# ProjectZKM/Ziren

Measured on AMD Instinct MI355X. Metric: shard-proofs/sec, higher is better.
Workload: dtype u32

## Files before the change

ziren_amd/csrc/host_ctx.hpp:

```cpp
#pragma once
static thread_local std::string g_err;

#define HIP_CHECK(expr)                                                                          \
  do {                                                                                           \
    hipError_t _e = (expr);                                                                      \
    if (_e != hipSuccess)                                                                        \
      throw std::runtime_error(std::string(#expr) + ": " + hipGetErrorString(_e) + " (" + __FILE__ + ":" + \
                               std::to_string(__LINE__) + ")");                                  \
  } while (0)
#define LAUNCH_CHECK() HIP_CHECK(hipGetLastError())
#define KLAUNCH(ctx, name, bytes, kernel, grid, block, lds, ...)                                        \
  do {                                                                                                   \
    (ctx)->flush_staged();                                                                               \
    if ((ctx)->kbegin(name, (double)(bytes))) {                                                          \
       \
      hipExtLaunchKernelGGL(kernel, grid, block, lds, (ctx)->cur, (ctx)->krecs.back().start,             \
                            (ctx)->krecs.back().stop, 0, __VA_ARGS__);                                   \
    } else {                                                                                             \
      hipLaunchKernelGGL(kernel, grid, block, lds, (ctx)->cur, __VA_ARGS__);                             \
    }                                                                                                    \
    LAUNCH_CHECK();                                                                                      \
  } while (0)

static inline int log2_strict(size_t n) {
// ... 78 lines not shown
  static constexpr size_t UP_SLAB_BYTES = (size_t)32 << 20;
  hipStream_t cur = nullptr;
  hipStream_t ev_dma = nullptr;
  struct Prefetched { size_t bytes; hipEvent_t landed; };
  std::map<const void*, Prefetched> prefetched;
  const uint32_t* events_on_device(const void* events, size_t bytes, uint32_t** owned) {
    *owned = nullptr;
    auto it = prefetched.find(events);
    if (it != prefetched.end()) {
      if (bytes > it->second.bytes) throw std::runtime_error("zkm_tracegen: more events asked for than zkm_events_upload_async copied");
      HIP_CHECK(hipStreamWaitEvent(stream, it->second.landed, 0));
      return (const uint32_t*)events;
    }
    uint32_t* d = (uint32_t*)alloc(std::max<size_t>(bytes, 4));
    *owned = d;
    if (bytes) HIP_CHECK(hipMemcpyAsync(d, events, bytes, hipMemcpyHostToDevice, stream));
    return d;
  }
  std::mutex mu;
  std::multimap<size_t, void*> free_list;
  std::map<void*, size_t> live;
  std::map<int, uint32_t*> tw_fwd, tw_inv;
  std::vector<std::pair<std::string, hipEvent_t>> marks;
  std::vector<hipEvent_t> event_pool;
  std::vector<std::string> timing_names;
  std::vector<float> timing_ms;
  struct KRec { const char* name; double bytes; hipEvent_t start, stop; };
  struct KStat { double ms = 0, bytes = 0; uint32_t calls = 0; };
  std::vector<KRec> krecs;
  std::map<std::string, KStat> kstats;
  int kernel_timing = 2;
  bool lde_overlap = !(getenv("ZKM_LDE_OVERLAP") && atoi(getenv("ZKM_LDE_OVERLAP")) == 0);
  bool rows_up_front = !(getenv("ZKM_ROWS_UP_FRONT") && atoi(getenv("ZKM_ROWS_UP_FRONT")) == 0);
  bool root_poll = !(getenv("ZKM_ROOT_POLL") && atoi(getenv("ZKM_ROOT_POLL")) == 0);
  int root_spin_before_yield = getenv("ZKM_ROOT_SPIN") ? atoi(getenv("ZKM_ROOT_SPIN")) : 4096;
  int root_sleep_ns = getenv("ZKM_ROOT_SLEEP_NS") ? atoi(getenv("ZKM_ROOT_SLEEP_NS")) : 0;
  bool host_wait_blocking = getenv("ZKM_HOST_WAIT") && !strcmp(getenv("ZKM_HOST_WAIT"), "blocking");
  int wait_sleep_ns = getenv("ZKM_WAIT_SLEEP_NS") ? atoi(getenv("ZKM_WAIT_SLEEP_NS")) : 20000;
  struct TimerSlack {
    long saved = -1;
    void tighten() {
      if (saved >= 0) return;
      saved = prctl(PR_GET_TIMERSLACK, 0, 0, 0, 0);
      if (saved >= 0) prctl(PR_SET_TIMERSLACK, 1000UL, 0, 0, 0);
    }
    ~TimerSlack() { if (saved >= 0) prctl(PR_SET_TIMERSLACK, (unsigned long)saved, 0, 0, 0); }
  };
  static void sleep_ns(long ns, TimerSlack& slack) {
    slack.tighten();
    timespec ts{0, ns};
    nanosleep(&ts, nullptr);
  }
  void sync(hipStream_t s) {
    if (!host_wait_blocking) { HIP_CHECK(hipStreamSynchronize(s)); return; }
    TimerSlack slack;
    for (int i = 0;; i++) {
      const hipError_t e = hipStreamQuery(s);
      if (e == hipSuccess) return;
      if (e != hipErrorNotReady) HIP_CHECK(e);
      if (i >= 4) sleep_ns(wait_sleep_ns, slack);
    }
  }
  std::map<uint64_t, std::vector<hipFunction_t>> quotient_fns;
  std::map<uint64_t, hipFunction_t> quotient_uniform_fns;
  std::map<uint64_t, hipFunction_t> perm_fns;
  std::vector<hipModule_t> modules;
// ... 345 lines not shown
```

ziren_amd/csrc/host_open.hpp:

```cpp
#pragma once
static E4 host_pow2k(E4 a, int k) { return kb::epow2k(a, k); }

struct Writer {
  uint32_t* dst;
  size_t cap, n = 0;
  Writer(uint32_t* d, size_t c) : dst(d), cap(d ? c : 0) {}
  void u(uint32_t v) { if (n < cap) dst[n] = v; n++; }
  void words(const uint32_t* p, size_t cnt) {
    if (n < cap) memcpy(dst + n, p, std::min(cnt, cap - n) * 4);
    n += cnt;
  }
  void ext(const E4& e) { words(e.c, 4); }
  size_t size() const { return n; }
};

struct RoundMat {
  const uint32_t* evals; size_t n; size_t width; uint32_t shift;
  const zkm_matrix* lde;
  int n_points;
  std::vector<E4> y[2];
  size_t col0 = 0;
};
struct Round { const zkm_pcs_data* data; std::vector<RoundMat> mats; };

// ... 121 lines not shown
    KLAUNCH(ctx, "scan", 0.0, stark::scan_totals, dim3((unsigned)(4 * scans.size())), dim3(stark::THREADS), 0, d);
    KLAUNCH(ctx, "scan", bytes, stark::scan_add_offsets, dim3(scans.back().blk_end), dim3(stark::THREADS), 0, d);
  }
}

struct ShardOpening {
  struct Loose {
    zkm_ctx* ctx;
    std::vector<void*> v;
    void disown(void* p) { v.erase(std::remove(v.begin(), v.end(), p), v.end()); }
    ~Loose() { for (void* p : v) ctx->release(p); }
  };
  struct Guard { zkm_ctx* c; std::vector<zkm_pcs_data*> d; ~Guard() { for (auto p : d) free_pcs_data(c, p); } };

  zkm_ctx* ctx;
  const zkm_pk* pk;
  zkm_main_data* md;
  const zkm_fri_config* fri;
  uint32_t num_pv_elts;
  zkm_challenger* ch;
  hipStream_t st;
  const int bl;
  const size_t nc;
  std::vector<ChipMeta> chips;
  Loose loose;
  std::vector<void*>& scratch;
  Guard guard;
  E4 perm_ch[2];
  uint32_t* d_pv = nullptr;
  std::vector<zkm_matrix> perm_traces;
  std::vector<E4> local_sums;
  std::vector<std::array<uint32_t, 14>> global_sums;
  zkm_pcs_data* perm_data = nullptr;
  std::vector<zkm_matrix> qchunks;
  std::vector<uint32_t> qshifts;
  zkm_pcs_data* quot_data = nullptr;
  E4 zeta;
  std::vector<Round> rounds;
  int log_max = 0;
  std::vector<E4*> ro = std::vector<E4*>(32, nullptr);
  const uint32_t** col_ptr_lde = nullptr;
  const uint32_t** col_ptr_eval = nullptr;
  uint32_t* col_mask = nullptr;
  std::vector<E4*> layers;
  std::vector<Tree> ftrees;
  std::vector<std::array<uint32_t, 8>> commits;
  E4 final_poly;
  uint32_t pow_witness = 0;
  std::vector<size_t> indices;
  const uint32_t* gathered = nullptr;
  std::vector<uint32_t> gathered_big;

  void* salloc(size_t bytes) { void* p = ctx->alloc(bytes); scratch.push_back(p); return p; }

  ShardOpening(zkm_ctx* ctx_, const zkm_pk* pk_, zkm_main_data* md_, const zkm_chip_desc* chips_in, const zkm_fri_config* fri_, uint32_t num_pv_elts_,
               zkm_challenger* ch_)
      : ctx(ctx_), pk(pk_), md(md_), fri(fri_), num_pv_elts(num_pv_elts_), ch(ch_), st(ctx_->stream), bl((int)fri_->log_blowup), nc(md_->order.size()),
        loose{ctx_, {}}, scratch(loose.v), guard{ctx_, {}} {
  for (size_t i = 0; i < nc; i++) chips.push_back(chip_meta(&chips_in[md->order[i]], md->traces[i].h, md->public_values.size()));
  for (size_t i = 0; i < nc; i++) {
    if (chips[i].desc->main_width != md->traces[i].w) throw std::runtime_error("chip main_width does not match its trace");
    if ((int)chips[i].desc->log_quotient_degree > bl) throw std::runtime_error("log_quotient_degree > log_blowup unsupported");
    if (chips[i].desc->prep_index >= 0 && (!pk->data || (size_t)chips[i].desc->prep_index >= pk->prep.size()))
      throw std::runtime_error("chip references a preprocessed trace the proving key does not hold");
  }
  if (bl < 1 || bl > 4) throw std::runtime_error("fri.log_blowup out of range (1..4)");
// ... 26 lines not shown
      if (chips[i].perm_ext_w > 0) d_blobs[i] = (uint32_t*)ctx->upload_staged(chips[i].desc->lookups, chips[i].desc->lookups_len * 4, &scratch);
    for (size_t i = 0; i < nc; i++) {
      const ChipMeta& c = chips[i];
      zkm_matrix& pt = perm_traces[i];
      pt.h = c.n; pt.w = (size_t)c.perm_ext_w * 4;
      pt.d = ctx->alloc_n<uint32_t>(std::max<size_t>(pt.h * pt.w, 1));
      scratch.push_back(pt.d);
      if (c.perm_ext_w > 0) {
        const uint32_t* prep = c.desc->prep_index >= 0 ? pk->prep[c.desc->prep_index].d : nullptr;
        launch_permutation_trace(ctx, c, (const uint32_t*)d_blobs[i], (const uint32_t*)md->traces[i].d, prep, perm_ch[0], (const E4*)d_bp, pt,
                                 [&](size_t bytes) { return salloc(bytes); }, scans);
        uint32_t* last = pt.d + (size_t)(c.perm_ext_w - 1) * 4 * c.n;
        for (int e = 0; e < 4; e++) sum_src.push_back(last + (size_t)e * c.n + (c.n - 1));
      } else {
        for (int e = 0; e < 4; e++) sum_src.push_back(nullptr);
      }
      if (c.desc->commit_scope_global) {
        const zkm_matrix& m = md->traces[i];
        for (int k = 0; k < 14; k++) sum_src.push_back(m.d + (m.w - 14 + k) * m.h + (m.h - 1));
      } else {
        for (int k = 0; k < 14; k++) sum_src.push_back(nullptr);
      }
    }
    launch_scans(ctx, scans, &scratch);
    const uint32_t* d_zero = (const uint32_t*)ctx->upload_staged("\0\0\0\0", 4, &scratch);
    for (auto& p : sum_src) if (!p) p = d_zero;
    const uint32_t** d_sum_src = (const uint32_t**)ctx->upload_staged(sum_src.data(), sum_src.size() * sizeof(void*), &scratch);
    uint32_t* d_sums = (uint32_t*)salloc(sum_src.size() * 4);
    KLAUNCH(ctx, "gather_words", 0.0, open::gather_words, dim3(div_up(sum_src.size(), open::THREADS)), dim3(open::THREADS), 0,
            (const uint32_t* const*)d_sum_src, sum_src.size(), d_sums);
    h_sums = ctx->download_async(d_sums, sum_src.size());
  }
  ctx->mark("permutation traces");
  perm_data = pcs_commit(ctx, perm_traces, {}, bl);
  guard.d.push_back(perm_data);
  perm_data->owned_evals = perm_traces;
  for (auto& m : perm_traces) loose.disown(m.d);
  ctx->mark("commit permutation");
  for (size_t i = 0; i < nc; i++) {
    for (int e = 0; e < 4; e++) local_sums[i].c[e] = h_sums[18 * i + e];
    if (chips[i].desc->commit_scope_global) {
      for (int k = 0; k < 14; k++) global_sums[i][k] = h_sums[18 * i + 4 + k];
    } else {
      for (int k = 0; k < 7; k++) { global_sums[i][k] = kb::to_monty(SEPTIC_X[k]); global_sums[i][7 + k] = kb::to_monty(SEPTIC_Y[k]); }
    }
  }
  chal::observe_slice(ch, perm_data->root, 8);
  for (size_t i = 0; i < nc; i++) {
    chal::observe_ext(ch, local_sums[i]);
    chal::observe_slice(ch, global_sums[i].data(), 14);
  }
  }

  void quotient_phase() {
  E4 alpha = chal::sample_ext(ch);
  std::vector<std::function<void()>> launches;
  for (size_t i = 0; i < nc; i++) {
    const ChipMeta& c = chips[i];
    const zkm_chip_desc* d = c.desc;
    int lqd = d->log_quotient_degree;
    int lq = c.log_n + lqd;
    size_t Q = (size_t)1 << lq;
    size_t nchunks = (size_t)1 << lqd;
    uint32_t* qbuf = ctx->alloc_n<uint32_t>(Q * 4);
    scratch.push_back(qbuf);
    size_t C = d->num_constraints;
    std::vector<E4> ap(std::max<size_t>(C, 1));
    E4 p = kb::eone();
    for (size_t k = 0; k < C; k++) { ap[C - 1 - k] = p; p = kb::emul(p, alpha); }
    E4* d_ap = (E4*)ctx->upload_staged(ap.data(), ap.size() * sizeof(E4), &scratch);
    uint32_t consts[32] = {0};
    for (int k = 0; k < 14; k++) consts[k] = global_sums[i][k];
    uint32_t w_q = kb::two_adic_generator(lq);
    uint32_t s_pow_n = kb::pow(kb::GEN, (uint64_t)c.n);
    uint32_t wr = kb::two_adic_generator(lqd), wp = kb::ONE;
    for (size_t k = 0; k < nchunks; k++) {
      consts[16 + k] = kb::sub(kb::mul(s_pow_n, wp), kb::ONE);
      consts[24 + k] = kb::inv(consts[16 + k]);
      wp = kb::mul(wp, wr);
    }
    uint32_t* d_consts = (uint32_t*)ctx->upload_staged(consts, sizeof consts, &scratch);
    static const uint32_t empty_prog[4] = {0, 1, 0, 1};
    uint32_t* d_prog = (uint32_t*)ctx->upload_staged(d->program_len ? d->program : empty_prog, std::max<size_t>(d->program_len, 4) * 4, &scratch);
    stark::QuotientArgs a;
    a.program = d_prog + 4;
    a.n_instr = d->program_len ? d->program[0] : 0;
    a.n_regs = d->program_len ? d->program[1] : 1;
    a.main_lde = md->data->ldes[i].d; a.main_stride = md->data->ldes[i].h;
    a.prep_lde = d->prep_index >= 0 ? pk->data->ldes[d->prep_index].d : nullptr;
    a.prep_stride = d->prep_index >= 0 ? pk->data->ldes[d->prep_index].h : 0;
    a.perm_lde = perm_data->ldes[i].d; a.perm_stride = perm_data->ldes[i].h;
    a.log_n = c.log_n; a.lqd = lqd;
    a.alpha_pows = d_ap; a.public_values = d_pv;
    a.perm_alpha = perm_ch[0]; a.perm_beta = perm_ch[1];
    a.local_sum = local_sums[i];
    a.consts = d_consts;
    a.w_q = w_q; a.g_inv = kb::inv(kb::two_adic_generator(c.log_n));
    a.out = qbuf;
// ... 4 lines not shown
    while (per_thread * bd > 64 * 1024 && bd > 64) bd >>= 1;
    size_t lds = per_thread * bd;
    if (lds > 152 * 1024) throw std::runtime_error(std::string("constraint program of chip ") + d->name + " needs too many registers");
    double qbytes = 4.0 * Q * (d->main_width + d->prep_width + 4.0 * c.perm_ext_w) + 16.0 * Q;
    auto fit = d->program_len ? ctx->quotient_fns.find(fnv1a(d->program, d->program_len)) : ctx->quotient_fns.end();
    const bool special = fit != ctx->quotient_fns.end();
    const std::vector<hipFunction_t>* fns = special ? &fit->second : nullptr;
    hipFunction_t uni_fn = nullptr;
    a.uniforms = nullptr;
    if (special) {
      auto uit = ctx->quotient_uniform_fns.find(fit->first);
      if (uit != ctx->quotient_uniform_fns.end()) {
        uni_fn = uit->second;
        a.uniforms = ctx->alloc_n<uint32_t>(stark::QUOTIENT_UNIFORM_WORDS);
        scratch.push_back(a.uniforms);
      }
    }
    launches.push_back([this, a, fns, uni_fn, Q, bd, lds, qbytes]() mutable {
      if (fns) {
        size_t arg_size = sizeof(a);
        void* config[] = {HIP_LAUNCH_PARAM_BUFFER_POINTER, &a, HIP_LAUNCH_PARAM_BUFFER_SIZE, &arg_size, HIP_LAUNCH_PARAM_END};
        ctx->flush_staged();
        if (uni_fn)
          HIP_CHECK(hipExtModuleLaunchKernel(uni_fn, 64, 1, 1, 64, 1, 1, 0, st, nullptr, config, nullptr, nullptr, 0));
        for (hipFunction_t fn : *fns) {
          const bool timed = ctx->kbegin("quotient", qbytes);
          HIP_CHECK(hipExtModuleLaunchKernel(fn, div_up(Q, 256) * 256, 1, 1, 256, 1, 1, 0, st, nullptr, config,
                                             timed ? ctx->krecs.back().start : nullptr, timed ? ctx->krecs.back().stop : nullptr, 0));
        }
      } else {
        KLAUNCH(ctx, "quotient", qbytes, stark::quotient_kernel, dim3(div_up(Q, bd)), dim3(bd), lds, a);
      }
    });
    uint32_t wqp = kb::ONE;
    for (size_t k = 0; k < nchunks; k++) {
      zkm_matrix m; m.h = c.n; m.w = 4; m.d = qbuf + k * 4 * c.n; m.owned = (k == 0);
      qchunks.push_back(m);
      qshifts.push_back(kb::mul(kb::GEN, wqp));
      wqp = kb::mul(wqp, w_q);
    }
    if (i == 0) { launches[0](); launches[0] = [] {}; }
  }
  for (auto& l : launches) l();
  ctx->mark("quotient values");
  quot_data = pcs_commit(ctx, qchunks, qshifts, bl);
  for (auto& m : qchunks) if (m.owned) { quot_data->owned_evals.push_back(m); loose.disown(m.d); }
  guard.d.push_back(quot_data);
  ctx->mark("commit quotient");
  chal::observe_slice(ch, quot_data->root, 8);
  zeta = chal::sample_ext(ch);
  }

  void opened_values() {
  if (pk->data) {
    Round r; r.data = pk->data;
    for (size_t j = 0; j < pk->prep.size(); j++)
      r.mats.push_back(RoundMat{pk->prep[j].d, pk->prep[j].h, pk->prep[j].w, kb::ONE, &pk->data->ldes[j], pk->local_only[j] ? 1 : 2, {}});
    rounds.push_back(r);
  }
  {
    Round r; r.data = md->data;
    for (size_t i = 0; i < nc; i++)
      r.mats.push_back(RoundMat{md->traces[i].d, md->traces[i].h, md->traces[i].w, kb::ONE, &md->data->ldes[i], chips[i].desc->local_only ? 1 : 2, {}});
    rounds.push_back(r);
    Round rp; rp.data = perm_data;
    for (size_t i = 0; i < nc; i++)
      rp.mats.push_back(RoundMat{perm_traces[i].d, perm_traces[i].h, perm_traces[i].w, kb::ONE, &perm_data->ldes[i], 2, {}});
    rounds.push_back(rp);
    Round rq; rq.data = quot_data;
    for (size_t i = 0; i < qchunks.size(); i++)
      rq.mats.push_back(RoundMat{qchunks[i].d, qchunks[i].h, 4, qshifts[i], &quot_data->ldes[i], 1, {}});
    rounds.push_back(rq);
  }
// ... 373 lines not shown
```

ziren_amd/csrc/host_pcs.hpp:

```cpp
#pragma once
struct LdeJob {
  const uint32_t* in; size_t n, w; uint32_t lde_shift; uint32_t* out;
  uint32_t* cflag = nullptr;
  bool uniform = false;
};

static void lde_batch_chunk(zkm_ctx* ctx, const std::vector<LdeJob>& jobs, int bl) {
  std::vector<size_t> order(jobs.size());
  std::iota(order.begin(), order.end(), 0);
  std::stable_sort(order.begin(), order.end(), [&](size_t a, size_t b) { return jobs[a].n > jobs[b].n; });
  std::vector<lde::Batch> hb(1);
  lde::Batch& b = hb[0];
  memset(&b, 0, sizeof b);
  b.log_blowup = bl;
  const size_t cosets = (size_t)1 << bl;
  size_t tmp1_words = 0, tmp2_words = 0;
  for (size_t oi : order) if (jobs[oi].n > ((size_t)1 << lde::LOG_ROW_MAX)) { tmp1_words += jobs[oi].n * jobs[oi].w; tmp2_words += (jobs[oi].n * jobs[oi].w) << bl; }
  uint32_t* tmp1 = tmp1_words ? ctx->alloc_n<uint32_t>(tmp1_words) : nullptr;
  uint32_t* tmp2 = tmp2_words ? ctx->alloc_n<uint32_t>(tmp2_words) : nullptr;
  size_t t1 = 0, t2 = 0;
  size_t big_cols = 0, fc = 0;
  for (size_t oi : order) if (jobs[oi].n > ((size_t)1 << lde::LOG_ROW_MAX) && !jobs[oi].cflag) big_cols += jobs[oi].w;
  uint32_t* cflags = big_cols ? ctx->alloc_n<uint32_t>(2 * big_cols) : nullptr;
  if (cflags) HIP_CHECK(hipMemsetAsync(cflags, 0, 2 * big_cols * sizeof(uint32_t), ctx->cur));
  uint32_t blk[4] = {0, 0, 0, 0};
  size_t lds_cols = 0, lds_small = 0;
  double bytes_inv = 0, bytes_rows = 0, bytes_fwd = 0, bytes_small = 0;
  int nm = 0;
  for (size_t p = 0; p < order.size();) {
    const size_t n = jobs[order[p]].n;
    const int k = log2_strict(n);
    const int lb = std::min(k, lde::LOG_ROW_MAX), la = k - lb;
    lde::Group& g = b.g[b.n_groups];
    g.la = la; g.lb = lb;
    g.logT = la ? std::min(14 - la, lb) : 0;
    g.first_mat = nm;
    g.w_N = kb::two_adic_generator(k + bl);
    g.n_inv = kb::inv(kb::to_monty((uint32_t)(n % kb::P)));
    g.twb_inv = lb > 0 ? ctx->twiddles(lb, true) : nullptr;
    g.twb_fwd = lb > 0 ? ctx->twiddles(lb, false) : nullptr;
    if (la) {
      g.twa_inv = ctx->twiddles_ct(la, true);
      g.twa_fwd = ctx->twiddles_ct(la, false);
      auto pw = ctx->pow_tables(k);
      g.pw_lo = pw.first; g.pw_hi = pw.second;
      g.tw_rows = ctx->row_twiddles(k);
    }
    uint32_t cols = 0;
    for (; p < order.size() && jobs[order[p]].n == n; p++) {
      const LdeJob& j = jobs[order[p]];
      lde::Mat& m = b.m[nm++];
      m.in = j.in; m.out = j.out; m.col0 = cols; m.w = (uint32_t)j.w; m.shift = j.lde_shift; m.uniform = j.uniform ? 1u : 0u;
      if (la) {
        m.tmp1 = tmp1 + t1; t1 += n * j.w;
        m.tmp2 = tmp2 + t2; t2 += (n * j.w) << bl;
        if (j.cflag) m.cflag = j.cflag;
        else { m.cflag = cflags + fc; fc += 2 * j.w; }
        auto ct = ctx->coset_tables(k, bl, j.lde_shift);
        m.twf = ct.twf; m.cs = ct.cs;
      }
      cols += (uint32_t)j.w;
    }
    g.n_cols = cols;
    g.n_mats = nm - g.first_mat;
    const double cells = (double)n * cols;
    if (la) {
      const size_t per_col = ((size_t)1 << lb) >> g.logT;
      blk[lde::K_COLS_INV] += (uint32_t)(per_col * cols);
      blk[lde::K_ROWS_BIG] += (uint32_t)(((size_t)1 << la) * cols);
      blk[lde::K_COLS_FWD] += (uint32_t)(per_col * cols * cosets);
      lds_cols = std::max(lds_cols, ((size_t)1 << la) * (((size_t)1 << g.logT) + 1) * 4);
      bytes_inv += 8.0 * cells; bytes_rows += 4.0 * cells * (1 + cosets); bytes_fwd += 8.0 * cells * cosets;
      for (int mi = (int)g.first_mat; mi < nm; mi++) if (b.m[mi].uniform) bytes_inv -= 8.0 * (double)n * b.m[mi].w;
    } else {
      blk[lde::K_ROWS_SMALL] += cols;
      const size_t B = (size_t)1 << lb;
      lds_small = std::max(lds_small, (2 * (B + (B >> 5)) + 64 + (B > 64 ? (B >> 6) : 1)) * 4);
      bytes_small += 4.0 * cells * (1 + cosets);
    }
    for (int q = 0; q < 4; q++) g.blk_end[q] = blk[q];
    b.n_groups++;
  }
  const lde::Batch* d = (const lde::Batch*)ctx->upload_staged(&b, sizeof b);
  if (blk[lde::K_COLS_INV]) {
    constexpr size_t B = (size_t)1 << lde::LOG_ROW_MAX;
    const size_t big_lds = (B + (B >> 5)) * 4;
    KLAUNCH(ctx, "lde_cols_inverse", bytes_inv, lde::lde_cols<false>, dim3(blk[lde::K_COLS_INV]), dim3(lde::THREADS), lds_cols, d);
    KLAUNCH(ctx, "lde_rows", bytes_rows, lde::lde_rows_big, dim3(blk[lde::K_ROWS_BIG]), dim3(lde::THREADS), big_lds, d);
    KLAUNCH(ctx, "lde_cols_forward", bytes_fwd, lde::lde_cols<true>, dim3(blk[lde::K_COLS_FWD]), dim3(lde::THREADS), lds_cols, d);
  }
  if (blk[lde::K_ROWS_SMALL])
    KLAUNCH(ctx, "lde_rows", bytes_small, lde::lde_rows, dim3(blk[lde::K_ROWS_SMALL]), dim3(lde::THREADS), lds_small, d);
  ctx->release_here(tmp1);
  ctx->release_here(tmp2);
  ctx->release_here(cflags);
  ctx->release_here((void*)d);
}

static void lde_batch(zkm_ctx* ctx, const std::vector<LdeJob>& all, int bl) {
  constexpr size_t SCRATCH_BUDGET_WORDS = ((size_t)12 << 30) / 4;
  std::vector<LdeJob> jobs;
  size_t scratch = 0;
  for (auto& j : all) {
    if (j.w == 0) continue;
    const size_t need = j.n > ((size_t)1 << lde::LOG_ROW_MAX) ? j.n * j.w + ((j.n * j.w) << bl) : 0;
    if (!jobs.empty() && ((int)jobs.size() == lde::MAX_MATS || scratch + need > SCRATCH_BUDGET_WORDS)) { lde_batch_chunk(ctx, jobs, bl); jobs.clear(); scratch = 0; }
    jobs.push_back(j);
    scratch += need;
  }
  if (!jobs.empty()) lde_batch_chunk(ctx, jobs, bl);
}

static void lde_columns(zkm_ctx* ctx, const uint32_t* in, size_t n, size_t w, int bl, uint32_t lde_shift, uint32_t* out) {
  lde_batch(ctx, {LdeJob{in, n, w, lde_shift, out}}, bl);
}

static const uint32_t** upload_ptrs(zkm_ctx* ctx, const std::vector<const uint32_t*>& ptrs) {
  return (const uint32_t**)ctx->upload_staged(ptrs.data(), ptrs.size() * sizeof(void*));
}

static bool compress_small_layer(zkm_ctx* ctx, Tree& t, int layer, size_t len, merkle::DevChallenger* d_ch = nullptr, kb::E4* d_beta = nullptr,
                                 uint32_t* h_root_slot = nullptr) {
  static const size_t LANES_MAX = getenv("ZKM_LANES_MAX") ? (size_t)atol(getenv("ZKM_LANES_MAX")) : 4096;
  const size_t TAIL = 64;
  if (len > LANES_MAX) {
    KLAUNCH(ctx, "compress_layer", 96.0 * len, merkle::compress_layer, dim3(div_up(len, merkle::THREADS)), dim3(merkle::THREADS), 0,
            (const uint32_t*)(t.digests + t.layer_off[layer] * 8), t.digests + t.layer_off[layer + 1] * 8, len,
            (const uint32_t* const*)nullptr, 0, (const uint32_t*)nullptr);
    return false;
  }
  if (len <= TAIL) {
    uint32_t* h_root = h_root_slot ? h_root_slot : (uint32_t*)ctx->pin_alloc(32);
    if (h_root) for (int k = 0; k < 8; k++) ((volatile uint32_t*)h_root)[k] = 0xffffffffu;
    KLAUNCH(ctx, "compress_tail", 96.0 * len, merkle::compress_tail_lanes, dim3(1), dim3(1024), 0, t.digests + t.layer_off[layer] * 8, len, h_root, d_ch, d_beta);
    t.h_root = h_root;
    return true;
  }
  KLAUNCH(ctx, "compress_small", 96.0 * len, merkle::compress_layer_lanes, dim3(div_up(len * 16, merkle::THREADS)), dim3(merkle::THREADS),
          0, (const uint32_t*)(t.digests + t.layer_off[layer] * 8), t.digests + t.layer_off[layer + 1] * 8, len);
  return false;
}

static inline void cpu_relax() {
#if defined(__x86_64__) || defined(__i386__)
  __builtin_ia32_pause();
#elif defined(__aarch64__)
  __asm__ __volatile__("yield");
// ... 147 lines not shown
              (const uint32_t*)(t.digests + t.layer_off[layer] * 8), t.digests + t.layer_off[layer + 1] * 8, len, (const uint32_t*)rowdig[len]);
      if (len == 1) break;
      continue;
    }
    const uint32_t** d = tables.count(len) ? tables[len].first : nullptr;
    struct { size_t n; size_t size() const { return n; } } ptrs{tables.count(len) ? tables[len].second : 0};
    if (d) wait_height(len);
    const uint32_t* prefix = nullptr;
    if (d && flag_tables.count(len) && flag_tables[len]) {
      uint32_t* out = prefixes + 32 * prefix_no++;
      KLAUNCH(ctx, "sponge_prefix", 0.0, merkle::sponge_prefix, dim3(1), dim3(64), 0, (const uint32_t* const*)flag_tables[len], (int)ptrs.size(), out);
      prefix = out;
    }
    KLAUNCH(ctx, "compress_layer", 96.0 * len + 4.0 * len * ptrs.size(), merkle::compress_layer, dim3(div_up(len, merkle::THREADS)),
            dim3(merkle::THREADS), 0, (const uint32_t*)(t.digests + t.layer_off[layer] * 8), t.digests + t.layer_off[layer + 1] * 8,
            len, (const uint32_t* const*)d, (int)ptrs.size(), prefix);
    if (len == 1) break;
  }
  for (auto d : to_free) ctx->release((void*)d);
  ctx->release(prefixes);
  ctx->release(rowdig_buf);
}

static void free_pcs_data(zkm_ctx* ctx, zkm_pcs_data* d) {
  if (!d) return;
  for (auto& m : d->ldes) ctx->release(m.d);
  for (auto& m : d->owned_evals) ctx->release(m.d);
  ctx->release(d->tree.digests);
  ctx->release(d->cflags);
  delete d;
}

static zkm_pcs_data* pcs_commit(zkm_ctx* ctx, const std::vector<zkm_matrix>& mats, const std::vector<uint32_t>& shifts,
                                int log_blowup) {
  zkm_pcs_data* d = new zkm_pcs_data();
  uint32_t* cflags = nullptr;
  try {
    d->log_blowup = log_blowup;
    for (size_t i = 0; i < mats.size(); i++) {
      const zkm_matrix& m = mats[i];
      zkm_matrix l;
      l.h = m.h << log_blowup;
      l.w = m.w;
      l.d = ctx->alloc_n<uint32_t>(l.h * l.w);
      d->ldes.push_back(l);
      d->evals.push_back(m.d);
      d->eval_heights.push_back(m.h);
      d->domain_shifts.push_back(shifts.empty() ? kb::ONE : shifts[i]);
    }
    auto shift_of = [&](size_t i) { return kb::mul(kb::GEN, kb::inv(d->domain_shifts[i])); };
    size_t flag_words = 0;
    for (auto& m : mats) if (m.h > ((size_t)1 << lde::LOG_ROW_MAX)) flag_words += 2 * m.w;
    cflags = flag_words ? ctx->alloc_n<uint32_t>(flag_words) : nullptr;
    if (cflags) HIP_CHECK(hipMemsetAsync(cflags, 0, flag_words * sizeof(uint32_t), ctx->stream));
    std::vector<const uint32_t*> col_flags(mats.size(), nullptr);
    {
      size_t off = 0;
      for (size_t i = 0; i < mats.size(); i++)
        if (mats[i].h > ((size_t)1 << lde::LOG_ROW_MAX)) { col_flags[i] = cflags + off; off += 2 * mats[i].w; }
    }
    auto job_of = [&](size_t i) { return LdeJob{mats[i].d, mats[i].h, mats[i].w, shift_of(i), d->ldes[i].d, const_cast<uint32_t*>(col_flags[i]), mats[i].uniform_rows}; };
    std::vector<char> extended(mats.size(), 0);
    size_t top = 0;
    for (auto& l : d->ldes) top = std::max(top, l.h);
    {
      const bool overlap = ctx->lde_overlap;
      std::vector<LdeJob> tall, rest;
      size_t rest_cells = 0;
      for (size_t i = 0; i < mats.size(); i++)
        if (!mats[i].ready || hipEventQuery(mats[i].ready) == hipSuccess) {
          (d->ldes[i].h == top ? tall : rest).push_back(job_of(i));
          if (d->ldes[i].h != top) rest_cells += mats[i].h * mats[i].w;
          extended[i] = 1;
        }
      if (overlap && !tall.empty() && rest_cells >= ((size_t)1 << 22)) {
        lde_batch(ctx, tall, log_blowup);
        ctx->side_begin();
        try { lde_batch(ctx, rest, log_blowup); } catch (...) { ctx->side_end(); ctx->side_join(); throw; }
        ctx->side_end();
      } else {
        tall.insert(tall.end(), rest.begin(), rest.end());
        lde_batch(ctx, tall, log_blowup);
      }
    }
    auto extend_height = [&](size_t lde_height) {
      if (lde_height < top) ctx->side_join();
      std::vector<LdeJob> jobs;
      for (size_t i = 0; i < mats.size(); i++) {
        if (extended[i] || d->ldes[i].h != lde_height) continue;
        wait_ready(ctx->stream, mats[i]);
        jobs.push_back(job_of(i));
        extended[i] = 1;
      }
      lde_batch(ctx, jobs, log_blowup);
    };
    const bool rows_up_front = ctx->rows_up_front && std::all_of(extended.begin(), extended.end(), [](char e) { return e != 0; });
    build_tree(ctx, d->ldes, d->tree, extend_height, &col_flags, rows_up_front);
    ctx->side_join();
    d->cflags = cflags;
    d->col_flags = col_flags;
    cflags = nullptr;
    for (size_t i = 0; i < mats.size(); i++)
      if (!extended[i]) throw std::runtime_error("pcs_commit: a matrix was not reached by the tree (internal error)");
    const uint32_t* h_root = d->tree.h_root ? d->tree.h_root : ctx->download_async(d->tree.node(d->tree.log_max, 0), 8);
    ctx->sync(ctx->stream);
    d->tree.h_root = nullptr;
    memcpy(d->root, h_root, 32);
  } catch (...) {
    ctx->cur = ctx->stream;
    try { ctx->side_join(); } catch (...) {}
    ctx->release(cflags);
    free_pcs_data(ctx, d);
    throw;
  }
  return d;
}
```

ziren_amd/csrc/lde.cuh:

```cuda
#pragma once
#include "kb31.cuh"
#include "gptr.cuh"

namespace lde {

constexpr int LOG_ROW_MAX = 13;
constexpr int THREADS = 512;

template <bool PAD>
__device__ __forceinline__ uint32_t phys(uint32_t i) { return PAD ? i + (i >> 5) : i; }

template <bool DIF, int R, bool LAZY = false>
__device__ __forceinline__ void butterflies(uint32_t (&x)[1 << R], uint32_t n, uint32_t s0, uint32_t lo, uint32_t logm2,
                                            const uint32_t* __restrict__ tw) {
  static_assert(!(DIF && LAZY), "the lazy form exists for the DIT butterfly only");
#pragma unroll
  for (int qq = 0; qq < R; qq++) {
    const uint32_t q = DIF ? qq : R - 1 - qq;
    const uint32_t s = s0 + q;
    const uint32_t half = 1u << (R - 1 - q);
    const uint32_t tbase = (n - (n >> s)) + lo;
#pragma unroll
    for (uint32_t j0 = 0; j0 < (1u << R); j0++) {
      if (j0 & half) continue;
// ... 110 lines not shown
  x0 = (uint32_t)kb::monty_reduce_signed(kb::mad_i64_i32(b, (int32_t)w, ar));
  x1 = (uint32_t)kb::monty_reduce_signed(kb::mad_i64_i32(b, -(int32_t)w, ar));
}
__device__ __forceinline__ uint32_t canonical(uint32_t lazy) {
  const uint32_t w = lazy + ((uint32_t)((int32_t)lazy >> 31) & (2u * kb::P));
  return kb::umin32(w, w - kb::P);
}

__device__ __forceinline__ void build_pow_table(uint32_t g, uint32_t* lo, uint32_t* hi, int nhi, uint32_t scale = kb::ONE) {
  uint32_t g64 = g;
  for (int i = 0; i < 6; i++) g64 = kb::sqr(g64);
  for (int i = threadIdx.x; i < 64 + nhi; i += blockDim.x) {
    if (i < 64) lo[i] = kb::mul(scale, kb::pow(g, (uint64_t)i));
    else hi[i - 64] = kb::pow(g64, (uint64_t)(i - 64));
  }
}
__device__ __forceinline__ uint32_t pow_lookup(const uint32_t* lo, const uint32_t* hi, uint32_t e) {
  return kb::mul(lo[e & 63], hi[e >> 6]);
}

constexpr int MAX_GROUPS = 24, MAX_MATS = 64;
enum { K_COLS_INV = 0, K_ROWS_BIG = 1, K_COLS_FWD = 2, K_ROWS_SMALL = 3 };

struct Mat {
  const uint32_t* in;
  uint32_t* out;
  uint32_t* tmp1;
  uint32_t* tmp2;
  const uint32_t* twf;
  const uint32_t* cs;
  uint32_t col0, w;
  uint32_t shift;
  uint32_t uniform;
  uint32_t* cflag;
};
struct Group {
  int la, lb, logT, pad;
  uint32_t n_cols, first_mat, n_mats, pad2;
  uint32_t blk_end[4];
  const uint32_t *twb_fwd, *twb_inv;
  const uint32_t *twa_fwd, *twa_inv;
  const uint32_t *pw_lo, *pw_hi;
  const uint32_t* tw_rows;
  uint32_t w_N, n_inv, pad3[2];
};
struct Batch {
  int n_groups, log_blowup;
  Group g[MAX_GROUPS];
  Mat m[MAX_MATS];
};

__device__ __forceinline__ const Group& find_group(const Batch* __restrict__ d, int which, uint32_t& local) {
  uint32_t gi = 0, start = 0;
  const uint32_t b = blockIdx.x;
  while (b >= d->g[gi].blk_end[which]) { start = d->g[gi].blk_end[which]; gi++; }
  local = b - start;
  return d->g[gi];
}
__device__ __forceinline__ const Mat& find_mat(const Batch* __restrict__ d, const Group& g, uint32_t col) {
  uint32_t mi = g.first_mat;
  while (col >= d->m[mi].col0 + d->m[mi].w) mi++;
  return d->m[mi];
}

template <bool FORWARD>
__global__ __launch_bounds__(THREADS) void lde_cols(const Batch* __restrict__ d) {
  extern __shared__ uint32_t lds[];
  uint32_t local;
  const Group& g = find_group(d, FORWARD ? K_COLS_FWD : K_COLS_INV, local);
  const int la = g.la, lb = g.lb, logT = g.logT, log_blowup = d->log_blowup;
  const int A = 1 << la, T = 1 << logT, TP = T + 1;
  const size_t B = (size_t)1 << lb, n = (size_t)A << lb;
  const uint32_t xb = local & ((1u << (lb - logT)) - 1);
  const uint32_t rest = local >> (lb - logT);
  const uint32_t col = FORWARD ? rest % g.n_cols : rest;
  const int z = FORWARD ? (int)(rest / g.n_cols) : 0;
  const Mat& m = find_mat(d, g, col);
  const size_t c = col - m.col0;
  const size_t t0 = (size_t)xb << logT;
  const uint32_t* src = (FORWARD ? m.tmp2 + (size_t)z * n * m.w : m.in) + c * n + t0;
  const uint32_t* __restrict__ tw = FORWARD ? g.twa_fwd : g.twa_inv;
  const int logTq = logT - 2;
  const int quads = (A << logT) >> 2;
  if (!FORWARD && m.uniform) {
    if (xb == 0 && threadIdx.x == 0) gp::store(m.cflag + 2 * c + 1, gp::load(m.in + c * n));
    return;
  }
  if (FORWARD && gp::load(m.cflag + 2 * c) == 0) {
    const uint32_t v0 = gp::load(m.cflag + 2 * c + 1);
    const uint32_t v = kb::umin32(v0, v0 - kb::P);
    uint32_t* dst = m.out + c * (n << log_blowup) + (size_t)kb::bitrev(z, log_blowup) * n;
    if (la < 2) {
      for (int u = threadIdx.x; u < (A << logT); u += blockDim.x)
        gp::store(dst + (size_t)kb::bitrev((uint32_t)(t0 + (u >> la)), lb) * A + (u & (A - 1)), v);
      return;
    }
    const int logAq = la - 2;
    for (int u0 = threadIdx.x; u0 < quads; u0 += blockDim.x) {
      const int t = u0 >> logAq, q = (u0 & ((1 << logAq) - 1)) << 2;
      gp::store(reinterpret_cast<uint4*>(dst + (size_t)kb::bitrev((uint32_t)(t0 + t), lb) * A + q), make_uint4(v, v, v, v));
    }
    return;
  }
  const uint32_t first_word = FORWARD ? 0u : gp::load(m.in + c * n);
  uint32_t differs = 0;
  for (int u0 = threadIdx.x; u0 < quads; u0 += 4 * blockDim.x) {
    uint4 v[4];
#pragma unroll
    for (int k = 0; k < 4; k++) {
      int u = u0 + k * blockDim.x;
      if (u < quads) v[k] = gp::load(reinterpret_cast<const uint4*>(src + (size_t)(u >> logTq) * B + ((u & ((1 << logTq) - 1)) << 2)));
    }
#pragma unroll
    for (int k = 0; k < 4; k++) {
      int u = u0 + k * blockDim.x;
      if (u < quads) {
        uint32_t* dd = lds + (u >> logTq) * TP + ((u & ((1 << logTq) - 1)) << 2);
        dd[0] = v[k].x; dd[1] = v[k].y; dd[2] = v[k].z; dd[3] = v[k].w;
        if (!FORWARD) differs |= (v[k].x ^ first_word) | (v[k].y ^ first_word) | (v[k].z ^ first_word) | (v[k].w ^ first_word);
      }
    }
  }
  if (!FORWARD) {
    if (__any(differs != 0) && (threadIdx.x & 63) == 0) gp::store(m.cflag + 2 * c, 1u);
    if (xb == 0 && threadIdx.x == 0) gp::store(m.cflag + 2 * c + 1, first_word);
  }
  __syncthreads();
  const bool fused_last = la >= 2 && (la & 3) == 1;
  lds_ntt_ct<false>(lds, la, logT, TP, tw, fused_last);
  const uint32_t* __restrict__ tw_last = tw + ((1u << (la - 1)) - 1);
  if (!FORWARD) {
    uint32_t* dst = m.tmp1 + c * n + t0;
    if (fused_last) {
      for (int u0 = threadIdx.x; u0 < (quads >> 1); u0 += blockDim.x) {
        const int rp = u0 >> logTq, qd = (u0 & ((1 << logTq) - 1)) << 2;
        const uint32_t* sp = lds + (2 * rp) * TP + qd;
        uint32_t x[4] = {sp[0], sp[1], sp[2], sp[3]}, y[4] = {sp[TP], sp[TP + 1], sp[TP + 2], sp[TP + 3]};
        const uint32_t w = gp::load(tw_last + rp);
#pragma unroll
        for (int k = 0; k < 4; k++) last_stage_ct(x[k], y[k], w);
        gp::store(reinterpret_cast<uint4*>(dst + (size_t)(2 * rp) * B + qd), make_uint4(x[0], x[1], x[2], x[3]));
        gp::store(reinterpret_cast<uint4*>(dst + (size_t)(2 * rp + 1) * B + qd), make_uint4(y[0], y[1], y[2], y[3]));
      }
      return;
    }
    for (int u0 = threadIdx.x; u0 < quads; u0 += blockDim.x) {
      const uint32_t* sp = lds + (u0 >> logTq) * TP + ((u0 & ((1 << logTq) - 1)) << 2);
      gp::store(reinterpret_cast<uint4*>(dst + (size_t)(u0 >> logTq) * B + ((u0 & ((1 << logTq) - 1)) << 2)), make_uint4(sp[0], sp[1], sp[2], sp[3]));
    }
  } else {
    uint32_t* dst = m.out + c * (n << log_blowup) + (size_t)kb::bitrev(z, log_blowup) * n;
    if (la < 2) {
      for (int u = threadIdx.x; u < (A << logT); u += blockDim.x) {
        const int t = u >> la, q = u & (A - 1);
        gp::store(dst + (size_t)kb::bitrev((uint32_t)(t0 + t), lb) * A + q, canonical(lds[q * TP + t]));
      }
      return;
    }
    const int logAq = la - 2;
    for (int u0 = threadIdx.x; u0 < quads; u0 += blockDim.x) {
      const int t = u0 >> logAq, q = (u0 & ((1 << logAq) - 1)) << 2;
      const uint32_t* sp = lds + q * TP + t;
      const size_t j0 = t0 + t;
      uint32_t x[4] = {sp[0], sp[TP], sp[2 * TP], sp[3 * TP]};
      if (fused_last) {
        last_stage_ct(x[0], x[1], gp::load(tw_last + (q >> 1)));
        last_stage_ct(x[2], x[3], gp::load(tw_last + (q >> 1) + 1));
      }
      gp::store(reinterpret_cast<uint4*>(dst + (size_t)kb::bitrev((uint32_t)j0, lb) * A + q),
                make_uint4(canonical(x[0]), canonical(x[1]), canonical(x[2]), canonical(x[3])));
    }
  }
}

__global__ __launch_bounds__(THREADS) void lde_rows(const Batch* __restrict__ d) {
  extern __shared__ uint32_t lds[];
  uint32_t col;
  const Group& g = find_group(d, K_ROWS_SMALL, col);
  const Mat& m = find_mat(d, g, col);
  const int lb = g.lb, log_blowup = d->log_blowup;
  const int B = 1 << lb;
  const int nhi = B > 64 ? (B >> 6) : 1;
  const int BP = B + (B >> 5);
  uint32_t* coef = lds;
  uint32_t* work = lds + BP;
  uint32_t* lo2 = work + BP;
  uint32_t* hi2 = lo2 + 64;
  const size_t c = col - m.col0;
  const uint32_t* src = m.in + c * B;
  const uint32_t* __restrict__ tw_fwd = g.twb_fwd;
  const uint32_t* __restrict__ tw_inv = g.twb_inv;
  for (int i = threadIdx.x; i < B; i += blockDim.x) coef[phys<true>(i)] = gp::load(src + i);
  __syncthreads();
  if (lb > 0) lds_ntt<true, true>(coef, lb, 0, 1, tw_inv);
  const int ncosets = 1 << log_blowup;
  uint32_t sj = m.shift;
  for (int j = 0; j < ncosets; j++) {
    __syncthreads();
    build_pow_table(sj, lo2, hi2, nhi, g.n_inv);
    __syncthreads();
    for (int i = threadIdx.x; i < B; i += blockDim.x)
      work[phys<true>(i)] = kb::mul(coef[phys<true>(i)], pow_lookup(lo2, hi2, kb::bitrev(i, lb)));
    __syncthreads();
    if (lb > 0) lds_ntt<false, true>(work, lb, 0, 1, tw_fwd);
    uint32_t* dst = m.out + c * ((size_t)B << log_blowup) + (size_t)kb::bitrev(j, log_blowup) * B;
    for (int i = threadIdx.x; i < B; i += blockDim.x) gp::store(dst + i, work[phys<true>(kb::bitrev(i, lb))]);
    sj = kb::mul(sj, g.w_N);
  }
}

__global__ __launch_bounds__(THREADS, 6) void lde_rows_big(const Batch* __restrict__ d) {
  constexpr uint32_t LB = LOG_ROW_MAX, B = 1u << LB, BP = B + (B >> 5);
  constexpr uint32_t G = B / THREADS;
  static_assert(G == 16 && LB == 13, "pass structure below is written for 8192 points on 512 threads");
  extern __shared__ uint32_t lds[];
  uint32_t* work = lds;
  uint32_t local;
  const Group& g = find_group(d, K_ROWS_BIG, local);
  const uint32_t la = g.la;
  const uint32_t tid = threadIdx.x;
  const uint32_t pr = local / g.n_cols;
  const uint32_t col = local - pr * g.n_cols;
  const Mat& m = find_mat(d, g, col);
  const size_t c = col - m.col0;
  const size_t n = (size_t)B << la;
  const uint32_t nmask = (uint32_t)n - 1;
  const uint32_t k1 = kb::bitrev(pr, la);
  if (gp::load(m.cflag + 2 * c) == 0) return;
  const uint32_t* src = m.tmp1 + c * n + (size_t)pr * B;
  const uint32_t* __restrict__ pw_lo = g.pw_lo;
  const uint32_t* __restrict__ pw_hi = g.pw_hi;
  auto pw = [&](uint32_t e) { return kb::mul(gp::load(pw_lo + (e & 1023)), gp::load(pw_hi + (e >> 10))); };

  const uint32_t* __restrict__ twr = g.tw_rows + (size_t)k1 * B;
  uint32_t x[16];
#pragma unroll
  for (uint32_t j = 0; j < 16; j++) x[j] = gp::load(src + tid + (j << 9));
  butterflies_ct<4, true>(x, 0, 0, twr);
#pragma unroll
  for (uint32_t j = 0; j < 16; j++) work[phys<true>(tid + (j << 9))] = x[j];
  __syncthreads();
  ntt_pass_ct<4, true>(work, LB, 4, twr);
  ntt_pass_ct<4, true>(work, LB, 8, twr);
  uint32_t keep[16];
#pragma unroll
  for (uint32_t k = 0; k < 8; k++) {
    const uint32_t gg = tid + (k << 9);
    const int32_t a = (int32_t)work[phys<true>(2 * gg)], b = (int32_t)work[phys<true>(2 * gg + 1)];
    const uint32_t w = gp::load(twr + (1u << 12) - 1 + gg);
    const int64_t ar = kb::mad_i64_i32_uniform(a, kb::ONE, 0);
    keep[2 * k] = (uint32_t)kb::monty_reduce_signed(kb::mad_i64_i32(b, (int32_t)w, ar));
    keep[2 * k + 1] = (uint32_t)kb::monty_reduce_signed(kb::mad_i64_i32(-b, (int32_t)w, ar));
  }
  const uint32_t st0 = pw((k1 * tid) & nmask), st_step = pw((k1 << 9) & nmask);
  const uint32_t ncosets = 1u << d->log_blowup;
  for (uint32_t j = 0; j < ncosets; j++) {
    const uint32_t* __restrict__ tw_fwd = m.twf + (size_t)j * B;
    const uint32_t t_first = gp::load(tw_fwd + B - 2);
    const uint32_t cj = gp::load(m.cs + (j << la) + k1);
    __syncthreads();
    uint32_t lt = tid;
    asm volatile("" : "+v"(lt));
#pragma unroll
    for (uint32_t k = 0; k < 8; k++) {
      const uint32_t gg = lt + (k << 9);
      const int64_t ar = kb::mad_i64_i32_uniform((int32_t)keep[2 * k], kb::ONE, 0);
      work[phys<true>(2 * gg)] = (uint32_t)kb::monty_reduce_signed(kb::mad_i64_i32_uniform((int32_t)keep[2 * k + 1], t_first, ar));
      work[phys<true>(2 * gg + 1)] = (uint32_t)kb::monty_reduce_signed(kb::mad_i64_i32_uniform((int32_t)keep[2 * k + 1], 0u - t_first, ar));
    }
    __syncthreads();
    ntt_pass<false, 4, true, true>(work, LB, 0, 1, 8, tw_fwd, lt);
    ntt_pass<false, 4, true, true>(work, LB, 0, 1, 4, tw_fwd, lt);
#pragma unroll
    for (uint32_t q = 0; q < 16; q++) x[q] = work[phys<true>(lt + (q << 9))];
    butterflies<false, 4, true>(x, B, 0, lt, 9, tw_fwd);
    uint32_t* dst = m.tmp2 + (size_t)j * n * m.w + c * n + (size_t)k1 * B;
    uint32_t t = kb::mul(st0, cj);
#pragma unroll
    for (uint32_t q = 0; q < 16; q++) {
      {
        const uint32_t r = (uint32_t)kb::monty_reduce_signed(kb::mad_i64_i32((int32_t)x[q], (int32_t)t, 0));
        gp::store(dst + lt + (q << 9), min(r, r + kb::P));
      }
      t = (uint32_t)kb::monty_reduce_signed(kb::mad_i64_i32_uniform((int32_t)t, st_step, 0));
    }
  }
}

__global__ void fill_stage_twiddles(uint32_t* tw, uint32_t w, int logn) {
// ... 50 lines not shown
```

Baseline: 9.401.

## Skip quotient for provably-zero permutation chips and copy identity LDE coset

Adds two shortcuts behind a default-on env flag. When a chip's trace has uniform rows, no preprocessed data and all-zero permutation column flags, the quotient kernel is replaced by a memset, with the flags downloaded to the host after the permutation commit. When an LDE coset shift equals one, that coset is written as a bit-reversed copy of the input instead of running the forward NTT. This removes NTT and quotient work, at the cost of an extra flag download and more branching in the kernels, and it relies on the zero-quotient reasoning being sound.

```diff
diff --git a/ziren_amd/csrc/host_ctx.hpp b/ziren_amd/csrc/host_ctx.hpp
--- a/ziren_amd/csrc/host_ctx.hpp
+++ b/ziren_amd/csrc/host_ctx.hpp
@@ -134,6 +134,7 @@
   int kernel_timing = 2;
   bool lde_overlap = !(getenv("ZKM_LDE_OVERLAP") && atoi(getenv("ZKM_LDE_OVERLAP")) == 0);
   bool rows_up_front = !(getenv("ZKM_ROWS_UP_FRONT") && atoi(getenv("ZKM_ROWS_UP_FRONT")) == 0);
+  bool quotient_shortcuts = !(getenv("ZKM_QUOTIENT_SHORTCUTS") && atoi(getenv("ZKM_QUOTIENT_SHORTCUTS")) == 0);
   bool root_poll = !(getenv("ZKM_ROOT_POLL") && atoi(getenv("ZKM_ROOT_POLL")) == 0);
   int root_spin_before_yield = getenv("ZKM_ROOT_SPIN") ? atoi(getenv("ZKM_ROOT_SPIN")) : 4096;
   int root_sleep_ns = getenv("ZKM_ROOT_SLEEP_NS") ? atoi(getenv("ZKM_ROOT_SLEEP_NS")) : 0;
diff --git a/ziren_amd/csrc/host_open.hpp b/ziren_amd/csrc/host_open.hpp
--- a/ziren_amd/csrc/host_open.hpp
+++ b/ziren_amd/csrc/host_open.hpp
@@ -177,6 +177,7 @@
   std::vector<E4> local_sums;
   std::vector<std::array<uint32_t, 14>> global_sums;
   zkm_pcs_data* perm_data = nullptr;
+  std::vector<uint32_t> perm_host_flags;
   std::vector<zkm_matrix> qchunks;
   std::vector<uint32_t> qshifts;
   zkm_pcs_data* quot_data = nullptr;
@@ -269,7 +270,9 @@
     h_sums = ctx->download_async(d_sums, sum_src.size());
   }
   ctx->mark("permutation traces");
-  perm_data = pcs_commit(ctx, perm_traces, {}, bl);
+  bool want_flags = false;
+  for (size_t i = 0; i < nc && ctx->quotient_shortcuts; i++) want_flags |= md->traces[i].uniform_rows && chips[i].desc->prep_index < 0;
+  perm_data = pcs_commit(ctx, perm_traces, {}, bl, want_flags ? &perm_host_flags : nullptr);
   guard.d.push_back(perm_data);
   perm_data->owned_evals = perm_traces;
   for (auto& m : perm_traces) loose.disown(m.d);
@@ -287,6 +290,17 @@
     chal::observe_ext(ch, local_sums[i]);
     chal::observe_slice(ch, global_sums[i].data(), 14);
   }
+  }
+
+  bool zero_quotient(size_t i) const {
+    if (!ctx->quotient_shortcuts || !md->traces[i].uniform_rows || chips[i].desc->prep_index >= 0) return false;
+    const size_t w = perm_traces[i].w;
+    if (w == 0) return true;
+    const uint32_t* cf = i < perm_data->col_flags.size() ? perm_data->col_flags[i] : nullptr;
+    if (!cf || perm_host_flags.empty()) return false;
+    const uint32_t* h = perm_host_flags.data() + (cf - perm_data->cflags);
+    for (size_t c = 0; c < w; c++) if (h[2 * c] != 0) return false;
+    return true;
   }
 
   void quotient_phase() {
@@ -301,6 +315,20 @@
     size_t nchunks = (size_t)1 << lqd;
     uint32_t* qbuf = ctx->alloc_n<uint32_t>(Q * 4);
     scratch.push_back(qbuf);
+    const bool zero = zero_quotient(i);
+    uint32_t wqp = kb::ONE;
+    for (size_t k = 0; k < nchunks; k++) {
+      zkm_matrix m; m.h = c.n; m.w = 4; m.d = qbuf + k * 4 * c.n; m.owned = (k == 0);
+      m.uniform_rows = zero;
+      qchunks.push_back(m);
+      qshifts.push_back(kb::mul(kb::GEN, wqp));
+      wqp = kb::mul(wqp, kb::two_adic_generator(lq));
+    }
+    if (zero) {
+      HIP_CHECK(hipMemsetAsync(qbuf, 0, Q * 4 * sizeof(uint32_t), st));
+      launches.push_back([] {});
+      continue;
+    }
     size_t C = d->num_constraints;
     std::vector<E4> ap(std::max<size_t>(C, 1));
     E4 p = kb::eone();
@@ -371,13 +399,6 @@
         KLAUNCH(ctx, "quotient", qbytes, stark::quotient_kernel, dim3(div_up(Q, bd)), dim3(bd), lds, a);
       }
     });
-    uint32_t wqp = kb::ONE;
-    for (size_t k = 0; k < nchunks; k++) {
-      zkm_matrix m; m.h = c.n; m.w = 4; m.d = qbuf + k * 4 * c.n; m.owned = (k == 0);
-      qchunks.push_back(m);
-      qshifts.push_back(kb::mul(kb::GEN, wqp));
-      wqp = kb::mul(wqp, w_q);
-    }
     if (i == 0) { launches[0](); launches[0] = [] {}; }
   }
   for (auto& l : launches) l();
diff --git a/ziren_amd/csrc/host_pcs.hpp b/ziren_amd/csrc/host_pcs.hpp
--- a/ziren_amd/csrc/host_pcs.hpp
+++ b/ziren_amd/csrc/host_pcs.hpp
@@ -3,7 +3,19 @@
   const uint32_t* in; size_t n, w; uint32_t lde_shift; uint32_t* out;
   uint32_t* cflag = nullptr;
   bool uniform = false;
+  int identity_coset = -1;
 };
+
+static int identity_coset_of(const zkm_ctx* ctx, size_t n, int bl, uint32_t lde_shift) {
+  if (!ctx->quotient_shortcuts) return -1;
+  const uint32_t w_N = kb::two_adic_generator(log2_strict(n) + bl);
+  uint32_t s = lde_shift;
+  for (int j = 0; j < (1 << bl); j++) {
+    if (s == kb::ONE) return j;
+    s = kb::mul(s, w_N);
+  }
+  return -1;
+}
 
 static void lde_batch_chunk(zkm_ctx* ctx, const std::vector<LdeJob>& jobs, int bl) {
   std::vector<size_t> order(jobs.size());
@@ -51,6 +63,7 @@
       const LdeJob& j = jobs[order[p]];
       lde::Mat& m = b.m[nm++];
       m.in = j.in; m.out = j.out; m.col0 = cols; m.w = (uint32_t)j.w; m.shift = j.lde_shift; m.uniform = j.uniform ? 1u : 0u;
+      m.identity_coset = j.identity_coset;
       if (la) {
         m.tmp1 = tmp1 + t1; t1 += n * j.w;
         m.tmp2 = tmp2 + t2; t2 += (n * j.w) << bl;
@@ -72,6 +85,7 @@
       lds_cols = std::max(lds_cols, ((size_t)1 << la) * (((size_t)1 << g.logT) + 1) * 4);
       bytes_inv += 8.0 * cells; bytes_rows += 4.0 * cells * (1 + cosets); bytes_fwd += 8.0 * cells * cosets;
       for (int mi = (int)g.first_mat; mi < nm; mi++) if (b.m[mi].uniform) bytes_inv -= 8.0 * (double)n * b.m[mi].w;
+      for (int mi = (int)g.first_mat; mi < nm; mi++) if (b.m[mi].identity_coset >= 0) bytes_rows -= 4.0 * (double)n * b.m[mi].w;
     } else {
       blk[lde::K_ROWS_SMALL] += cols;
       const size_t B = (size_t)1 << lb;
@@ -112,7 +126,7 @@
 }
 
 static void lde_columns(zkm_ctx* ctx, const uint32_t* in, size_t n, size_t w, int bl, uint32_t lde_shift, uint32_t* out) {
-  lde_batch(ctx, {LdeJob{in, n, w, lde_shift, out}}, bl);
+  lde_batch(ctx, {LdeJob{in, n, w, lde_shift, out, nullptr, false, identity_coset_of(ctx, n, bl, lde_shift)}}, bl);
 }
 
 static const uint32_t** upload_ptrs(zkm_ctx* ctx, const std::vector<const uint32_t*>& ptrs) {
@@ -326,7 +340,7 @@
 }
 
 static zkm_pcs_data* pcs_commit(zkm_ctx* ctx, const std::vector<zkm_matrix>& mats, const std::vector<uint32_t>& shifts,
-                                int log_blowup) {
+                                int log_blowup, std::vector<uint32_t>* host_flags = nullptr) {
   zkm_pcs_data* d = new zkm_pcs_data();
   uint32_t* cflags = nullptr;
   try {
@@ -353,7 +367,8 @@
       for (size_t i = 0; i < mats.size(); i++)
         if (mats[i].h > ((size_t)1 << lde::LOG_ROW_MAX)) { col_flags[i] = cflags + off; off += 2 * mats[i].w; }
     }
-    auto job_of = [&](size_t i) { return LdeJob{mats[i].d, mats[i].h, mats[i].w, shift_of(i), d->ldes[i].d, const_cast<uint32_t*>(col_flags[i]), mats[i].uniform_rows}; };
+    auto job_of = [&](size_t i) { return LdeJob{mats[i].d, mats[i].h, mats[i].w, shift_of(i), d->ldes[i].d, const_cast<uint32_t*>(col_flags[i]), mats[i].uniform_rows,
+                                                identity_coset_of(ctx, mats[i].h, log_blowup, shift_of(i))}; };
     std::vector<char> extended(mats.size(), 0);
     size_t top = 0;
     for (auto& l : d->ldes) top = std::max(top, l.h);
@@ -397,7 +412,9 @@
     for (size_t i = 0; i < mats.size(); i++)
       if (!extended[i]) throw std::runtime_error("pcs_commit: a matrix was not reached by the tree (internal error)");
     const uint32_t* h_root = d->tree.h_root ? d->tree.h_root : ctx->download_async(d->tree.node(d->tree.log_max, 0), 8);
+    const uint32_t* h_flags = host_flags && d->cflags ? ctx->download_async((const uint32_t*)d->cflags, flag_words) : nullptr;
     ctx->sync(ctx->stream);
+    if (host_flags) host_flags->assign(h_flags, h_flags + (h_flags ? flag_words : 0));
     d->tree.h_root = nullptr;
     memcpy(d->root, h_root, 32);
   } catch (...) {
diff --git a/ziren_amd/csrc/lde.cuh b/ziren_amd/csrc/lde.cuh
--- a/ziren_amd/csrc/lde.cuh
+++ b/ziren_amd/csrc/lde.cuh
@@ -166,6 +166,7 @@
   uint32_t col0, w;
   uint32_t shift;
   uint32_t uniform;
+  int32_t identity_coset;
   uint32_t* cflag;
 };
 struct Group {
@@ -212,7 +213,8 @@
   const Mat& m = find_mat(d, g, col);
   const size_t c = col - m.col0;
   const size_t t0 = (size_t)xb << logT;
-  const uint32_t* src = (FORWARD ? m.tmp2 + (size_t)z * n * m.w : m.in) + c * n + t0;
+  const bool copy = FORWARD && z == m.identity_coset;
+  const uint32_t* src = (FORWARD && !copy ? m.tmp2 + (size_t)z * n * m.w : m.in) + c * n + t0;
   const uint32_t* __restrict__ tw = FORWARD ? g.twa_fwd : g.twa_inv;
   const int logTq = logT - 2;
   const int quads = (A << logT) >> 2;
@@ -260,8 +262,8 @@
     if (xb == 0 && threadIdx.x == 0) gp::store(m.cflag + 2 * c + 1, first_word);
   }
   __syncthreads();
-  const bool fused_last = la >= 2 && (la & 3) == 1;
-  lds_ntt_ct<false>(lds, la, logT, TP, tw, fused_last);
+  const bool fused_last = !copy && la >= 2 && (la & 3) == 1;
+  if (!copy) lds_ntt_ct<false>(lds, la, logT, TP, tw, fused_last);
   const uint32_t* __restrict__ tw_last = tw + ((1u << (la - 1)) - 1);
   if (!FORWARD) {
     uint32_t* dst = m.tmp1 + c * n + t0;
@@ -287,7 +289,7 @@
     if (la < 2) {
       for (int u = threadIdx.x; u < (A << logT); u += blockDim.x) {
         const int t = u >> la, q = u & (A - 1);
-        gp::store(dst + (size_t)kb::bitrev((uint32_t)(t0 + t), lb) * A + q, canonical(lds[q * TP + t]));
+        gp::store(dst + (size_t)kb::bitrev((uint32_t)(t0 + t), lb) * A + q, canonical(lds[(copy ? kb::bitrev((uint32_t)q, la) : q) * TP + t]));
       }
       return;
     }
@@ -297,6 +299,10 @@
       const uint32_t* sp = lds + q * TP + t;
       const size_t j0 = t0 + t;
       uint32_t x[4] = {sp[0], sp[TP], sp[2 * TP], sp[3 * TP]};
+      if (copy) {
+#pragma unroll
+        for (int k = 0; k < 4; k++) x[k] = lds[kb::bitrev((uint32_t)(q + k), la) * TP + t];
+      }
       if (fused_last) {
         last_stage_ct(x[0], x[1], gp::load(tw_last + (q >> 1)));
         last_stage_ct(x[2], x[3], gp::load(tw_last + (q >> 1) + 1));
@@ -326,10 +332,19 @@
   const uint32_t* __restrict__ tw_inv = g.twb_inv;
   for (int i = threadIdx.x; i < B; i += blockDim.x) coef[phys<true>(i)] = gp::load(src + i);
   __syncthreads();
+  if (m.identity_coset >= 0) {
+    uint32_t* dst = m.out + c * ((size_t)B << log_blowup) + (size_t)kb::bitrev((uint32_t)m.identity_coset, log_blowup) * B;
+    for (int i = threadIdx.x; i < B; i += blockDim.x) {
+      const uint32_t v = coef[phys<true>(kb::bitrev(i, lb))];
+      gp::store(dst + i, kb::umin32(v, v - kb::P));
+    }
+    __syncthreads();
+  }
   if (lb > 0) lds_ntt<true, true>(coef, lb, 0, 1, tw_inv);
   const int ncosets = 1 << log_blowup;
   uint32_t sj = m.shift;
   for (int j = 0; j < ncosets; j++) {
+    if (j == m.identity_coset) { sj = kb::mul(sj, g.w_N); continue; }
     __syncthreads();
     build_pow_table(sj, lo2, hi2, nhi, g.n_inv);
     __syncthreads();
@@ -389,6 +404,7 @@
   const uint32_t st0 = pw((k1 * tid) & nmask), st_step = pw((k1 << 9) & nmask);
   const uint32_t ncosets = 1u << d->log_blowup;
   for (uint32_t j = 0; j < ncosets; j++) {
+    if ((int32_t)j == m.identity_coset) continue;
     const uint32_t* __restrict__ tw_fwd = m.twf + (size_t)j * B;
     const uint32_t t_first = gp::load(tw_fwd + B - 2);
     const uint32_t cj = gp::load(m.cs + (j << la) + k1);
```

New measurement: 23.87, median of 6. +153.9%, better.
